# liuzhenboo/Stereo-Visual-Odometry

Hardware: AMD Instinct MI355X
Metric: stereo frames/sec on KITTI-00 1241x376; LK-kernel achieved HBM GB/s vs peak (higher is better)
Workload: dtype u8; 1 GPU; S0 synthetic KITTI-like stereo sequence 1241x376 (config #2 stand-in), FAST+LK track_mode LK_stereof2f_pnp, batched frame pairs (256 per step, 4 distinct chunks cycled), frames resident in HBM for `value`; `m1` (--full) = host-resident frames, H2D included; pairs_ok_last_step=256, parallelism=1 GPU

## Files before the change

include/svo_abi.h:

```cpp
#ifndef SVO_ABI_H
#define SVO_ABI_H

#include <stdint.h>

#ifdef __cplusplus
extern "C" {
#endif

#define SVO_ABI_VERSION 9

#define SVO_OK                 0
#define SVO_ERR_ARG           -1
#define SVO_ERR_HIP           -2
#define SVO_ERR_NOMEM         -3
#define SVO_ERR_STATE         -4
#define SVO_FAIL_FEW_KEYPOINTS 1
#define SVO_FAIL_FEW_TRACKS    2
#define SVO_FAIL_INLIER_RATIO  3
#define SVO_FAIL_ROTATION_GATE 4
#define SVO_FAIL_TRANSL_GATE   5
#define SVO_FAIL_CAPACITY      6

#define SVO_MEM_HOST   0
#define SVO_MEM_DEVICE 1

typedef struct svo_ctx svo_ctx;

typedef struct { float x, y; } svo_pt2f;
typedef struct { float x, y, z; } svo_pt3f;
typedef struct {
    float x, y, size, angle, response;
    int32_t octave, class_id;
} svo_keypoint;

typedef struct {
    int32_t width, height;
    int32_t max_keypoints;
    int32_t max_batch;
    int32_t num_slots;
    int32_t fast_threshold;
    int32_t num_features_tracking;
    int32_t iterations;
    float   reproj_err;
    float   confidence;
    double  feature_match_error;
    double  inlier_rate;
    double  min_move2, max_move2;
    double  P1[12], P2[12];
    int32_t track_mode;
    int32_t orb_nfeatures;
    float   orb_scale_factor;
    int32_t orb_nlevels;
    int32_t orb_ini_th, orb_min_th;
    int32_t lk_accum;
    int32_t fast_keep_strongest;
} svo_config;

#define SVO_MODE_LK  0
#define SVO_MODE_ORB 1
#define SVO_LK_ACCUM_EXACT 0
#define SVO_LK_ACCUM_SSE2  1
#define SVO_LK_ACCUM_SIMD128 2
#define SVO_LK_ACCUM_SSE2_LEGACY 3

typedef struct {
    double rvec[3], tvec[3], R[9];
    int32_t n_inliers, ransac_iters, best_iter, lm_iters, ok, _pad;
} svo_pnp_result;

typedef struct {
    int32_t ok;
    int32_t fail_stage;
    int32_t n_prev_kps, n_cur_kps, n_tracked, n_inliers;
    int32_t ransac_iters, lm_iters;
    double  rvec[3], tvec[3], R[9];
    double  T_rel_inv[16];
    double  pose[16];
} svo_step_result;

int         svo_abi_version(void);
int         svo_config_bytes(void);
void        svo_default_config(svo_config *cfg, int width, int height);
int         svo_device_count(int *n);
int         svo_create(const svo_config *cfg, int device, svo_ctx **out);
void        svo_destroy(svo_ctx *ctx);
const char *svo_last_error(const svo_ctx *ctx);
int         svo_set_stream(svo_ctx *ctx, void *hip_stream);
int         svo_sync(svo_ctx *ctx);
int         svo_wait_stream(svo_ctx *ctx, void *hip_stream);
int         svo_signal_stream(svo_ctx *ctx, void *hip_stream);
int         svo_signal_stream_inputs(svo_ctx *ctx, void *hip_stream);
int         svo_num_levels(const svo_ctx *ctx);


int svo_fast_detect(svo_ctx *ctx, const uint8_t *img, int pitch, int mem, int threshold,
                    int nonmax, svo_keypoint *out, int cap, int *n_out);

int svo_build_pyramid(svo_ctx *ctx, int slot, const uint8_t *img, int pitch, int mem);
int svo_read_pyramid_level(svo_ctx *ctx, int slot, int level, uint8_t *out, int out_pitch, int mem,
                           int *w, int *h);

int svo_lk_track(svo_ctx *ctx, int slot_prev, int slot_next, const svo_pt2f *prev_pts, int n,
                 svo_pt2f *next_pts, uint8_t *status, int mem);

int svo_circular_match(svo_ctx *ctx, int slot_prevL, int slot_prevR, int slot_curL, int slot_curR,
                       const svo_pt2f *t1_left, int n, svo_pt2f *out_t1_left,
                       svo_pt2f *out_t1_right, svo_pt2f *out_t2_right, svo_pt2f *out_t2_left,
                       int *m_out, int mem);

int svo_triangulate(svo_ctx *ctx, const double P1[12], const double P2[12], const svo_pt2f *x1,
                    const svo_pt2f *x2, int n, svo_pt3f *out, int mem);

int svo_pnp_ransac(svo_ctx *ctx, const svo_pt3f *obj, const svo_pt2f *img, int n, const double K[9],
                   int iterations, float reproj_err, double confidence, svo_pnp_result *res,
                   uint8_t *inlier_mask, int mem);

int svo_orb_extract(svo_ctx *ctx, const uint8_t *img, int pitch, int mem, svo_keypoint *kps, uint8_t *desc,
                    int cap, int *n_out, int *per_level);
int svo_orb_read_level(svo_ctx *ctx, int level, uint8_t *out, int *w, int *h);
int svo_orb_read_candidates(svo_ctx *ctx, int level, float *out4, int cap, int *n_out);

int svo_match_hamming(svo_ctx *ctx, const uint8_t *query, int nq, const uint8_t *train, int nt, int32_t *train_idx,
                      float *distance, int mem);


int svo_add_frame(svo_ctx *ctx, const uint8_t *left, const uint8_t *right, int pitch, int mem,
                  svo_step_result *res);
int svo_reset(svo_ctx *ctx);
int svo_get_pose(svo_ctx *ctx, double pose[16]);
int svo_set_pose(svo_ctx *ctx, const double pose[16]);

int svo_track_batch(svo_ctx *ctx, const uint8_t *left_frames, const uint8_t *right_frames,
                    int pitch, int64_t frame_stride, int n_frames, const double *pose0,
                    svo_step_result *results, int results_mem);

int svo_set_overlap(svo_ctx *ctx, int on);
int svo_wait_results(svo_ctx *ctx);

int svo_host_alloc(svo_ctx *ctx, size_t bytes, void **out);
int svo_host_free(svo_ctx *ctx, void *p);
int svo_upload_frames(svo_ctx *ctx, int buf, const uint8_t *left_frames, const uint8_t *right_frames,
                      int pitch, int64_t frame_stride, int n_frames);
int svo_upload_frames_at(svo_ctx *ctx, int buf, int first_slot, const uint8_t *left_frames, const uint8_t *right_frames,
                         int pitch, int64_t frame_stride, int n_frames);
int svo_wait_upload(svo_ctx *ctx, int buf);
int svo_track_uploaded(svo_ctx *ctx, int buf, int n_frames, const double *pose0,
                       svo_step_result *results, int results_mem);
#define SVO_CONTINUE_CHAIN       1
#define SVO_CONTINUE_CARRY_FRAME 2
int svo_track_uploaded_async(svo_ctx *ctx, int buf, int n_frames, const double *pose0, int continue_chain);
int svo_collect_results(svo_ctx *ctx, svo_step_result *results, int n_pairs);
int svo_results_ready(svo_ctx *ctx, int *n_pairs);

int svo_get_frame_keypoints(svo_ctx *ctx, int side, svo_keypoint *kps, uint8_t *descriptors, int cap, int *n_out);
int svo_get_last_tracks(svo_ctx *ctx, svo_pt2f *t1_left, svo_pt2f *t1_right, svo_pt2f *t2_right,
                        svo_pt2f *t2_left, uint8_t *inlier, int cap, int *n_out);
int svo_get_batch_tracks(svo_ctx *ctx, int pair, svo_pt2f *t1_left, svo_pt2f *t1_right, svo_pt2f *t2_right,
                         svo_pt2f *t2_left, uint8_t *inlier, int cap, int *n_out);

int svo_streams_create(svo_ctx *ctx, int n_streams);
int svo_streams_count(const svo_ctx *ctx, int *n_streams);
int svo_streams_step(svo_ctx *ctx, const int32_t *stream_ids, int m, const uint8_t *left_frames,
                     const uint8_t *right_frames, int pitch, int64_t frame_stride, int mem,
                     svo_step_result *results, int results_mem);
int svo_streams_reset(svo_ctx *ctx, int stream_id);
int svo_streams_get_pose(svo_ctx *ctx, int stream_id, double pose[16]);
int svo_streams_set_pose(svo_ctx *ctx, int stream_id, const double pose[16]);
int svo_streams_get_tracks(svo_ctx *ctx, int item, svo_pt2f *t1_left, svo_pt2f *t1_right, svo_pt2f *t2_right,
                           svo_pt2f *t2_left, uint8_t *inlier, int cap, int *n_out);

#define SVO_INTERP_NEAREST 0
#define SVO_INTERP_LINEAR  1
int svo_scale_projection(const double P[12], double inv_x, double inv_y, int interp, double P_out[12]);
int svo_resize(svo_ctx *ctx, const uint8_t *src, int sw, int sh, int spitch, int64_t sstride,
               uint8_t *dst, int dw, int dh, int dpitch, int64_t dstride, int n_frames,
               int interp, double fx, double fy, int mem);
int svo_ingest_create(svo_ctx *ctx, int src_width, int src_height, int interp, double fx, double fy);
int svo_ingest_info(const svo_ctx *ctx, int *src_width, int *src_height, int *interp, double *inv_x, double *inv_y);
int svo_ingest_add_frame(svo_ctx *ctx, const uint8_t *left, const uint8_t *right, int pitch, int mem, svo_step_result *res);
int svo_ingest_track_batch(svo_ctx *ctx, const uint8_t *lefts, const uint8_t *rights, int pitch, int64_t frame_stride,
                           int n_frames, const double *pose0, svo_step_result *results, int results_mem);
int svo_ingest_streams_step(svo_ctx *ctx, const int32_t *stream_ids, int m, const uint8_t *lefts, const uint8_t *rights,
                            int pitch, int64_t frame_stride, int mem, svo_step_result *results, int results_mem);
// ... 57 lines not shown
```

stereo-visual-odometry_amd/binding.py:

```python
import ctypes as C
import os
import subprocess

import numpy as np

_HERE = os.path.dirname(os.path.abspath(__file__))
_LIB = None

MEM_HOST, MEM_DEVICE = 0, 1

KP_DTYPE = np.dtype([("x", "<f4"), ("y", "<f4"), ("size", "<f4"), ("angle", "<f4"),
                     ("response", "<f4"), ("octave", "<i4"), ("class_id", "<i4")])


class SvoError(RuntimeError):
    pass


class Config(C.Structure):
    _fields_ = [("width", C.c_int32), ("height", C.c_int32), ("max_keypoints", C.c_int32),
                ("max_batch", C.c_int32), ("num_slots", C.c_int32), ("fast_threshold", C.c_int32),
                ("num_features_tracking", C.c_int32), ("iterations", C.c_int32),
                ("reproj_err", C.c_float), ("confidence", C.c_float),
                ("feature_match_error", C.c_double), ("inlier_rate", C.c_double),
# ... 230 lines not shown
        return rc

    def sync(self):
        self._check(self.lib.svo_sync(self.h))

    def set_stream(self, stream_handle):
        self._check(self.lib.svo_set_stream(self.h, C.c_void_p(stream_handle)))
        self._stream_handle = int(stream_handle or 0)

    def wait_stream(self, stream_handle):
        self._check(self.lib.svo_wait_stream(self.h, C.c_void_p(stream_handle)))

    def signal_stream(self, stream_handle):
        self._check(self.lib.svo_signal_stream(self.h, C.c_void_p(stream_handle)))

    def signal_stream_inputs(self, stream_handle):
        self._check(self.lib.svo_signal_stream_inputs(self.h, C.c_void_p(stream_handle)))

    def _order_in(self, t):
        import torch
        other = torch.cuda.current_stream(t.device).cuda_stream
        if other and other == getattr(self, "_stream_handle", 0):
            return False
        self.wait_stream(other)
        return True

    def _order_out(self, t):
        import torch
        other = torch.cuda.current_stream(t.device).cuda_stream
        if other and other == getattr(self, "_stream_handle", 0):
            return
        self.signal_stream(other)

    @property
    def num_levels(self):
        return self.lib.svo_num_levels(self.h)

    def set_overlap(self, on=True):
        self._check(self.lib.svo_set_overlap(self.h, int(on)))

    def wait_results(self):
        self._check(self.lib.svo_wait_results(self.h))

    def enable_timing(self, on=True):
        self._check(self.lib.svo_enable_timing(self.h, int(on)))

    def get_timing(self):
        names = (C.c_char_p * 64)()
        ms = (C.c_float * 64)()
        n = self.lib.svo_get_timing(self.h, names, ms, 64)
        return [(names[i].decode(), float(ms[i])) for i in range(n)]

    def _img(self, img, shape=None):
        shape = shape or (self.height, self.width)
        assert tuple(img.shape) == tuple(shape), (tuple(img.shape), shape)
        if isinstance(img, np.ndarray):
            assert img.dtype == np.uint8 and img.strides[1] == 1
            return C.c_void_p(img.ctypes.data), int(img.strides[0]), MEM_HOST
        assert img.element_size() == 1 and img.stride(1) == 1
        return C.c_void_p(img.data_ptr()), int(img.stride(0)), (MEM_DEVICE if img.is_cuda else MEM_HOST)

    def fast_detect(self, img, threshold=20, nonmax=True, cap=None):
        cap = cap or self.cfg.max_keypoints
        p, pitch, mem = self._img(img)
        out = np.zeros(cap, dtype=KP_DTYPE)
        n = C.c_int(0)
        self._check(self.lib.svo_fast_detect(self.h, p, pitch, mem, int(threshold), int(bool(nonmax)),
                                             C.c_void_p(out.ctypes.data), cap, C.byref(n)))
        return out[:n.value].copy()

    def build_pyramid(self, slot, img):
        p, pitch, mem = self._img(img)
        self._check(self.lib.svo_build_pyramid(self.h, int(slot), p, pitch, mem))

    def read_pyramid_level(self, slot, level):
        w, h = C.c_int(0), C.c_int(0)
        self._check(self.lib.svo_read_pyramid_level(self.h, slot, level, None, 0, MEM_HOST,
                                                    C.byref(w), C.byref(h)))
        out = np.zeros((h.value, w.value), np.uint8)
        self._check(self.lib.svo_read_pyramid_level(self.h, slot, level, C.c_void_p(out.ctypes.data),
                                                    w.value, MEM_HOST, C.byref(w), C.byref(h)))
        return out

    def lk_track(self, slot_prev, slot_next, pts):
        if isinstance(pts, np.ndarray):
            pts = np.ascontiguousarray(pts, np.float32).reshape(-1, 2)
            n = pts.shape[0]
            out = np.zeros((n, 2), np.float32)
            st = np.zeros(n, np.uint8)
        else:
            import torch
            n = pts.shape[0]
            out = torch.zeros((n, 2), dtype=torch.float32, device=pts.device)
            st = torch.zeros(n, dtype=torch.uint8, device=pts.device)
            self._order_in(st)
        pi, mem = _ptr(pts)
        po, _ = _ptr(out)
        ps, _ = _ptr(st)
        self._check(self.lib.svo_lk_track(self.h, slot_prev, slot_next, pi, n, po, ps, mem))
        if mem == MEM_DEVICE:
            self._order_out(st)
        return out, st

    def circular_match(self, slots, t1_left):
        if isinstance(t1_left, np.ndarray):
            t1_left = np.ascontiguousarray(t1_left, np.float32).reshape(-1, 2)
            n = t1_left.shape[0]
            outs = [np.zeros((max(n, 1), 2), np.float32) for _ in range(4)]
        else:
            import torch
            n = t1_left.shape[0]
            outs = [torch.zeros((max(n, 1), 2), dtype=torch.float32, device=t1_left.device) for _ in range(4)]
            self._order_in(outs[0])
        pi, mem = _ptr(t1_left)
        m = C.c_int(0)
        self._check(self.lib.svo_circular_match(self.h, *[int(s) for s in slots], pi, n,
                                                *[_ptr(o)[0] for o in outs], C.byref(m), mem))
        return [o[:m.value] for o in outs]

    def triangulate(self, P1, P2, x1, x2):
        P1 = np.ascontiguousarray(P1, np.float64).reshape(12)
        P2 = np.ascontiguousarray(P2, np.float64).reshape(12)
        if isinstance(x1, np.ndarray):
            x1 = np.ascontiguousarray(x1, np.float32).reshape(-1, 2)
            x2 = np.ascontiguousarray(x2, np.float32).reshape(-1, 2)
            out = np.zeros((x1.shape[0], 3), np.float32)
        else:
            import torch
            out = torch.zeros((x1.shape[0], 3), dtype=torch.float32, device=x1.device)
            self._order_in(out)
        p1, mem = _ptr(x1)
        p2, _ = _ptr(x2)
        self._check(self.lib.svo_triangulate(self.h, C.c_void_p(P1.ctypes.data), C.c_void_p(P2.ctypes.data),
                                             p1, p2, x1.shape[0], _ptr(out)[0], mem))
        if mem == MEM_DEVICE:
            self._order_out(out)
        return out

    def pnp_ransac(self, obj, img, K, iterations=500, reproj_err=0.5, confidence=0.99):
        K = np.ascontiguousarray(K, np.float64).reshape(9)
        if isinstance(obj, np.ndarray):
            obj = np.ascontiguousarray(obj, np.float32).reshape(-1, 3)
            img = np.ascontiguousarray(img, np.float32).reshape(-1, 2)
            mask = np.zeros(max(obj.shape[0], 1), np.uint8)
        else:
            import torch
            mask = torch.zeros(max(obj.shape[0], 1), dtype=torch.uint8, device=obj.device)
            self._order_in(mask)
        n = obj.shape[0]
        res = PnPResult()
        po, mem = _ptr(obj)
        conf = float(np.float32(confidence))
        self._check(self.lib.svo_pnp_ransac(self.h, po, _ptr(img)[0], n, C.c_void_p(K.ctypes.data),
                                            int(iterations), C.c_float(reproj_err), C.c_double(conf),
                                            C.byref(res), _ptr(mask)[0], mem))
        if mem == MEM_DEVICE:
            self._order_out(mask)
            mask = mask.cpu().numpy()
        return dict(ok=res.ok, rvec=np.array(res.rvec), tvec=np.array(res.tvec),
                    R=np.array(res.R).reshape(3, 3), n_inliers=res.n_inliers,
                    ransac_iters=res.ransac_iters, best_iter=res.best_iter, lm_iters=res.lm_iters,
                    mask=np.asarray(mask[:n]).copy())

    def set_pose_refine(self, mode, rounds=4, iters=10, sigma_px=1.0, min_inliers=6):
        names = {"off": REFINE_OFF, "none": REFINE_OFF, "reproj": REFINE_REPROJ}
        m = names[mode] if isinstance(mode, str) and mode in names else mode
# ... 488 lines not shown
```

stereo-visual-odometry_amd/csrc/fast.hip:

```cpp
#include "svo_device.h"
#include "svo_kernels.h"

namespace svo {

constexpr int kTileW = 64, kTileH = 16, kHalo = 4;
constexpr int kRawW = kTileW + 2 * kHalo;
constexpr int kRawH = kTileH + 2 * kHalo;
constexpr int kScW = kTileW + 2;
constexpr int kScH = kTileH + 2;

__device__ __forceinline__ void load_circle(const uint8_t *c, int d[16], int v)
{
    constexpr int P = kRawW;
    d[0] = v - c[3 * P];       d[1] = v - c[3 * P + 1];   d[2] = v - c[2 * P + 2];   d[3] = v - c[P + 3];
    d[4] = v - c[3];           d[5] = v - c[-P + 3];      d[6] = v - c[-2 * P + 2];  d[7] = v - c[-3 * P + 1];
    d[8] = v - c[-3 * P];      d[9] = v - c[-3 * P - 1];  d[10] = v - c[-2 * P - 2]; d[11] = v - c[-P - 3];
    d[12] = v - c[-3];         d[13] = v - c[P - 3];      d[14] = v - c[2 * P - 2];  d[15] = v - c[3 * P - 1];
}

__device__ __forceinline__ bool has_arc9(unsigned m16)
{
    unsigned m = m16 | (m16 << 16);
    unsigned a = m & (m >> 1);
    unsigned b = a & (a >> 2);
// ... 106 lines not shown
#pragma unroll
                for (int hb = 0; hb < 2; hb++) {
                    auto half = [&](uint32_t w) { return __builtin_bit_cast(s16x2, (hb ? w >> 8 : w) & 0x00FF00FFu); };
                    const s16x2 v = half(C), u = half(U), d = half(D), l = half(Lv), rr = half(Rv);
                    const s16x2 mnA = __builtin_elementwise_min(u, d), mxA = __builtin_elementwise_max(u, d);
                    const s16x2 mnB = __builtin_elementwise_min(l, rr), mxB = __builtin_elementwise_max(l, rr);
                    const s16x2 dark = __builtin_elementwise_min(v - mnA, v - mnB);
                    const s16x2 bright = __builtin_elementwise_min(mxA - v, mxB - v);
                    sgn[hb] = __builtin_bit_cast(uint32_t, __builtin_elementwise_max(dark, bright) - T1);
                }
                const uint32_t dead = ((sgn[0] >> 15) & 1u) | ((sgn[1] >> 14) & 2u) | ((sgn[0] >> 29) & 4u) | ((sgn[1] >> 28) & 8u);
                const int gy = y0 - 1 + sy, gxb = x0 - 1 + sxb;
                const int lo = max(max(0, -sxb), 3 - gxb), hi = min(min(4, kScW - sxb), a.w - 3 - gxb);
                const uint32_t inside = (hi > lo && gy >= 3 && gy < a.h - 3) ? ((1u << hi) - 1u) & ~((1u << lo) - 1u) : 0u;
                m4 = ~dead & inside;
            }
            const int lane = threadIdx.x;
            const unsigned long long lt = (1ull << lane) - 1ull;
            const unsigned long long b0 = __ballot(m4 & 1u), b1 = __ballot(m4 & 2u), b2 = __ballot(m4 & 4u), b3 = __ballot(m4 & 8u);
            const int c0 = __popcll(b0), c1 = __popcll(b1), c2 = __popcll(b2), c3 = __popcll(b3);
            if (c0 + c1 + c2 + c3) {
                int base = 0;
                if (lane == 0) base = atomicAdd(&n_cand, c0 + c1 + c2 + c3);
                base = __builtin_amdgcn_readfirstlane(base);
                const int pos = sy * kScW + sxb;
                if (m4 & 1u) cand[base + __popcll(b0 & lt)] = (uint16_t)pos;
                if (m4 & 2u) cand[base + c0 + __popcll(b1 & lt)] = (uint16_t)(pos + 1);
                if (m4 & 4u) cand[base + c0 + c1 + __popcll(b2 & lt)] = (uint16_t)(pos + 2);
                if (m4 & 8u) cand[base + c0 + c1 + c2 + __popcll(b3 & lt)] = (uint16_t)(pos + 3);
            }
        }
    }
    __syncthreads();
    const int nc = n_cand;
    for (int i0 = 0; i0 < nc; i0 += 256) {
        const int i = i0 + tid;
        const int pos = i < nc ? cand[i] : 0;
        const int sy = pos / kScW, sx = pos - sy * kScW;
        const bool corner = i < nc && fast_arc(&raw[(sy + kHalo - 1) * kRawW + sx + kHalo - 1], a.thr);
        if (a.nms) list_push(corner, pos, corners, &n_corner);
        else if (corner) sc[pos] = 1;
    }
    __syncthreads();
    if (a.nms) {
        const int nk = n_corner;
        for (int i = tid; i < nk; i += 256) {
            const int pos = corners[i];
            const int sy = pos / kScW, sx = pos - sy * kScW;
            sc[pos] = (uint8_t)fast_corner_score(&raw[(sy + kHalo - 1) * kRawW + sx + kHalo - 1], a.thr);
        }
        __syncthreads();
    }

#pragma unroll
    for (int j = 0; j < kTileH / 4; j++) {
        int ly = threadIdx.y + 4 * j, lx = threadIdx.x;
        int gx = x0 + lx, gy = y0 + ly;
        const uint8_t *p = &sc[(ly + 1) * kScW + lx + 1];
        int s = p[0];
        if (a.nms && s) {
            bool keep = s > p[-1] && s > p[1] && s > p[-kScW - 1] && s > p[-kScW] && s > p[-kScW + 1] &&
                        s > p[kScW - 1] && s > p[kScW] && s > p[kScW + 1];
            if (!keep) s = 0;
        }
        bool inimg = gx < a.w && gy < a.h;
        if (!inimg) s = 0;
        unsigned long long m = __ballot(s != 0);
        if (inimg) score[(int64_t)gy * a.spitch + gx] = (uint8_t)s;
        if (threadIdx.x == 0 && m && gy < a.h) atomicAdd(&rowcount[gy], __popcll(m));
    }
}

__global__ __launch_bounds__(256) void fast_emit_kernel(FastArgs a)
{
    const int b = blockIdx.y;
    const int y = blockIdx.x * 4 + (threadIdx.x >> 6);
    const int lane = threadIdx.x & 63;
    if (y >= a.h) return;
    const uint8_t *score = a.score + (int64_t)b * a.score_stride + (int64_t)y * a.spitch;
    const int *rowcount = a.rowcount + (int64_t)b * a.rowcount_stride;
    int mine = rowcount[y];
    bool last = (y == a.h - 1);
    if (mine == 0 && !last) return;
    int part = 0;
    for (int r = lane; r < y; r += 64) part += rowcount[r];
    int off = wave_sum_i32(part);
    if (last && lane == 0) a.n_out[b] = off + mine;
    if (mine == 0) return;
    float2 *xy = a.kp_xy + (int64_t)b * a.kp_stride;
    float *resp = a.kp_resp + (int64_t)b * a.kp_stride;
    for (int x = lane; x < ((a.w + 63) & ~63); x += 64) {
        int s = x < a.w ? score[x] : 0;
        unsigned long long m = __ballot(s != 0);
        if (s) {
            int idx = off + __popcll(m & ((1ull << lane) - 1ull));
            if (idx < a.cap) {
                xy[idx] = make_float2((float)x, (float)y);
                resp[idx] = a.nms ? (float)s : 0.f;
            }
        }
        off += __popcll(m);
    }
}

__global__ __launch_bounds__(1024) void fast_keep_strongest_kernel(FastArgs a, int keep)
{
    __shared__ int hist[256];
    __shared__ int wave_eq[16], wave_kp[16];
    __shared__ int s_t, s_need_eq, s_eq_base, s_out_base;
    const int b = blockIdx.x, tid = threadIdx.x, lane = tid & 63, wv = tid >> 6;
    const int n = a.n_out[b];
    if (n <= keep || n > a.cap) return;
    float2 *xy = a.kp_xy + (int64_t)b * a.kp_stride;
    float *resp = a.kp_resp + (int64_t)b * a.kp_stride;
    if (tid < 256) hist[tid] = 0;
    __syncthreads();
    for (int i = tid; i < n; i += 1024) atomicAdd(&hist[min(255, max(0, (int)resp[i]))], 1);
    __syncthreads();
    if (tid == 0) {
        int above = 0, t = 255;
        for (; t > 0; t--) {
            if (above + hist[t] >= keep) break;
            above += hist[t];
        }
        s_t = t; s_need_eq = keep - above; s_eq_base = 0; s_out_base = 0;
    }
    __syncthreads();
    const int t = s_t, need_eq = s_need_eq;
    for (int start = 0; start < n; start += 1024) {
        const int i = start + tid;
        const bool in = i < n;
        const float2 p = in ? xy[i] : make_float2(0.f, 0.f);
        const float r = in ? resp[i] : 0.f;
        const int ri = (int)r;
        const bool eq = in && ri == t;
        const unsigned long long me = __ballot(eq);
        if (lane == 0) wave_eq[wv] = __popcll(me);
        __syncthreads();
        int eq_pre = s_eq_base, eq_tot = 0;
        for (int q = 0; q < 16; q++) { const int c = wave_eq[q]; if (q < wv) eq_pre += c; eq_tot += c; }
        const int eq_rank = eq_pre + __popcll(me & ((1ull << lane) - 1ull));
        const bool kp = in && (ri > t || (eq && eq_rank < need_eq));
        const unsigned long long mk = __ballot(kp);
        if (lane == 0) wave_kp[wv] = __popcll(mk);
        __syncthreads();
        int kp_pre = s_out_base, kp_tot = 0;
        for (int q = 0; q < 16; q++) { const int c = wave_kp[q]; if (q < wv) kp_pre += c; kp_tot += c; }
        if (kp) {
            const int dst = kp_pre + __popcll(mk & ((1ull << lane) - 1ull));
            xy[dst] = p; resp[dst] = r;
        }
        __syncthreads();
        if (tid == 0) { s_eq_base += eq_tot; s_out_base += kp_tot; }
        __syncthreads();
    }
    if (tid == 0) a.n_out[b] = keep;
}

void launch_fast_keep_strongest(const FastArgs &a, int batch, int keep, hipStream_t st)
{
    if (keep <= 0 || batch <= 0 || !a.nms) return;
    hipLaunchKernelGGL(fast_keep_strongest_kernel, dim3(batch), dim3(1024), 0, st, a, keep);
}

constexpr int kBucketLdsCells = 3072;

__device__ __forceinline__ void bucket_count(int *cnt, int cell, bool flag)
{
    const int lane = threadIdx.x & 63;
    const int prev = __shfl_up(cell, 1);
    const bool head = lane == 0 || prev != cell;
    const unsigned long long H = __ballot(head), F = __ballot(flag);
    if (head && cell >= 0) {
        const unsigned long long below = (1ull << lane) - 1ull;
        const unsigned long long after = lane == 63 ? 0ull : H & ~(below | (1ull << lane));
        const unsigned long long upto = after ? (1ull << (__ffsll((long long)after) - 1)) - 1ull : ~0ull;
        const int c = __popcll(F & upto & ~below);
        if (c) atomicAdd(&cnt[4 * cell], c);
    }
}

template <bool kLds>
__global__ __launch_bounds__(1024) void fast_bucket_kernel(BucketArgs a)
{
// ... 128 lines not shown
```

stereo-visual-odometry_amd/csrc/pyramid.hip:

```cpp
#include "svo_device.h"
#include "svo_kernels.h"

namespace svo {

__device__ __forceinline__ const uint8_t *src_image(const PyrArgs &a, int b)
{
    if (a.img2) return ((b & 1) ? a.img2 : a.img) + (int64_t)(b >> 1) * a.img_stride;
    return a.img + (int64_t)b * a.img_stride;
}

__global__ __launch_bounds__(256) void pyr_copy0_kernel(PyrArgs a)
{
    const int b = blockIdx.z, y = blockIdx.y * blockDim.y + threadIdx.y;
    const int w = a.g.w[0];
    if (y >= a.g.h[0]) return;
    const uint8_t *src = src_image(a, b) + (int64_t)y * a.pitch;
    uint8_t *dst = a.slots + (int64_t)b * a.slot_stride + a.g.origin[0] + (int64_t)y * a.g.pitch[0];
    const int x = (blockIdx.x * blockDim.x + threadIdx.x) * 16;
    if (x >= w) return;
    if (x + 16 <= w && ((uintptr_t)(src + x) & 15) == 0) {
        *(uint4 *)(dst + x) = *(const uint4 *)(src + x);
    } else {
        for (int q = 0; q < 16 && x + q < w; q++) dst[x + q] = src[x + q];
    }
}

constexpr int kBorderRows = 16;
constexpr int kFrameRowsPerWg = 4, kSidePasses = 4;
__host__ __device__ inline int border_top_groups() { return 2 * kPad / kFrameRowsPerWg; }
__host__ __device__ inline int border_side_groups(int h) { return (h + kBorderRows * kSidePasses - 1) / (kBorderRows * kSidePasses); }
__global__ __launch_bounds__(256) void pyr_border_kernel(PyrArgs a, int l)
{
    const int b = blockIdx.y;
    const int w = a.g.w[l], h = a.g.h[l], pitch = a.g.pitch[l];
    uint8_t *lvl = a.slots + (int64_t)b * a.slot_stride + a.g.origin[l];
    if ((int)blockIdx.x < border_top_groups()) {
        for (int q = 0; q < kFrameRowsPerWg; q++) {
            const int gidx = blockIdx.x * kFrameRowsPerWg + q;
            const int py = gidx < kPad ? gidx - kPad : h + (gidx - kPad);
            const uint8_t *src = lvl + (int64_t)refl101(py, h) * pitch;
            uint8_t *dst = lvl + (int64_t)py * pitch;
            for (int px = ((int)threadIdx.x << 2) - kPad; px < w + kPad; px += 1024) {
                uint32_t v = 0;
                if (px >= 0 && px + 4 <= w) v = *(const uint32_t *)(src + px);
                else {
#pragma unroll
                    for (int k = 0; k < 4; k++) v |= (uint32_t)src[refl101(min(px + k, w + kPad - 1), w)] << (8 * k);
                }
                if (px + 4 <= w + kPad) *(uint32_t *)(dst + px) = v;
                else for (int k = 0; px + k < w + kPad; k++) dst[px + k] = (uint8_t)(v >> (8 * k));
            }
        }
        return;
    }
    const int sgroup = blockIdx.x - border_top_groups();
    if (w >= 2 * kPad) {
        static_assert(kBorderRows == 16 && kPad == 32, "256 threads = 16 rows x 16 dwords");
        typedef uint32_t u32_unaligned __attribute__((aligned(1)));
        const int k = threadIdx.x & 15, r = threadIdx.x >> 4;
        const int px = k < 8 ? -kPad + 4 * k : w + 4 * (k - 8);
        const int c0 = k < 8 ? kPad - 3 - 4 * k : w - 5 - 4 * (k - 8);
        for (int q = 0; q < kSidePasses; q++) {
            const int py = (sgroup * kSidePasses + q) * kBorderRows + r;
            if (py >= h) return;
            uint8_t *row = lvl + (int64_t)py * pitch;
            const uint32_t v = *(const u32_unaligned *)(row + c0);
            *(u32_unaligned *)(row + px) = __builtin_amdgcn_perm(0u, v, 0x00010203u);
        }
    } else {
        const int t = threadIdx.x & 63;
        const int px = t < kPad ? t - kPad : w + (t - kPad);
        const int sx = refl101(px, w);
        for (int q = 0; q < kSidePasses; q++)
            for (int r = threadIdx.x >> 6; r < kBorderRows; r += 4) {
                const int py = (sgroup * kSidePasses + q) * kBorderRows + r;
                if (py >= h) return;
                uint8_t *row = lvl + (int64_t)py * pitch;
                row[px] = row[sx];
            }
    }
}

__global__ __launch_bounds__(256) void pyr_down_kernel(PyrArgs a, int l)
{
    const int b = blockIdx.z, y = blockIdx.y * blockDim.y + threadIdx.y;
    const int w = a.g.w[l];
    if (y >= a.g.h[l]) return;
    const int sp = a.g.pitch[l - 1];
    uint8_t *slot = a.slots + (int64_t)b * a.slot_stride;
    const uint8_t *src = slot + a.g.origin[l - 1];
    uint8_t *dst = slot + a.g.origin[l] + (int64_t)y * a.g.pitch[l];
    const int x0 = (blockIdx.x * blockDim.x + threadIdx.x) * 4;
    if (x0 >= w) return;
    int acc[4] = {0, 0, 0, 0};
#pragma unroll
    for (int r = 0; r < 5; r++) {
        const uint32_t *row = (const uint32_t *)(src + (int64_t)(2 * y + r - 2) * sp + 2 * x0 - 4);
        const uint32_t d0 = row[0], d1 = row[1], d2 = row[2], d3 = row[3];
        int s[16];
#pragma unroll
        for (int j = 0; j < 4; j++) {
            s[j] = (d0 >> (8 * j)) & 255; s[4 + j] = (d1 >> (8 * j)) & 255;
            s[8 + j] = (d2 >> (8 * j)) & 255; s[12 + j] = (d3 >> (8 * j)) & 255;
        }
        const int wv = (r == 2) ? 6 : ((r == 1 || r == 3) ? 4 : 1);
#pragma unroll
        for (int q = 0; q < 4; q++) {
            const int c = 4 + 2 * q;
            const int hs = s[c] * 6 + (s[c - 1] + s[c + 1]) * 4 + s[c - 2] + s[c + 2];
            acc[q] += hs * wv;
        }
    }
    uint32_t out = 0;
#pragma unroll
    for (int q = 0; q < 4; q++) out |= (uint32_t)((acc[q] + 128) >> 8) << (8 * q);
    if (x0 + 4 <= w) *(uint32_t *)(dst + x0) = out;
    else for (int q = 0; x0 + q < w; q++) dst[x0 + q] = (uint8_t)(out >> (8 * q));
}

__global__ __launch_bounds__(256) void pyr_read_level_kernel(PyrGeom g, const uint8_t *slot, int l,
                                                              uint8_t *out, int out_pitch)
{
    int x = blockIdx.x * 256 + threadIdx.x, y = blockIdx.y;
    if (x >= g.w[l]) return;
    out[(int64_t)y * out_pitch + x] = slot[g.origin[l] + (int64_t)y * g.pitch[l] + x];
}

void launch_pyramid(const PyrArgs &a, int batch, hipStream_t st)
{
    dim3 blk(256, 1, 1);
    auto shape = [](int lanes_per_row, int rows, dim3 &grid, dim3 &block, int batch) {
        const int bx = lanes_per_row < 256 ? lanes_per_row : 256, by = 256 / bx;
        block = dim3(bx, by, 1);
        grid = dim3((lanes_per_row + bx - 1) / bx, (rows + by - 1) / by, batch);
    };
    {
        dim3 g, bk;
        shape((a.g.w[0] + 15) / 16, a.g.h[0], g, bk, batch);
        hipLaunchKernelGGL(pyr_copy0_kernel, g, bk, 0, st, a);
    }
    for (int l = 0; l < a.g.nlevels; l++) {
        if (l > 0) {
            dim3 g, bk;
            shape((a.g.w[l] + 3) / 4, a.g.h[l], g, bk, batch);
            hipLaunchKernelGGL(pyr_down_kernel, g, bk, 0, st, a, l);
        }
        dim3 gb(border_top_groups() + border_side_groups(a.g.h[l]), batch, 1);
        hipLaunchKernelGGL(pyr_border_kernel, gb, blk, 0, st, a, l);
    }
}

// ... 9 lines not shown
```

stereo-visual-odometry_amd/csrc/svo_abi.hip:

```cpp
#include <algorithm>
#include <cmath>
#include <cstdio>
#include <cstring>
#include <ctime>
#include <new>
#include <vector>
#include "abi_io.h"

using namespace svo;

namespace svo {
int dev_alloc_raw(svo_ctx *ctx, void **out, size_t bytes)
{
    *out = nullptr;
    if (bytes == 0) bytes = 1;
    if (ctx->arena.planning) {
        ctx->arena.plan.emplace_back(out, ctx->arena.planned);
        ctx->arena.planned += align_up(bytes, kDevAlign);
        return SVO_OK;
    }
    SVO_HIP(hipMalloc(out, bytes));
    ctx->arena.extra.push_back(*out);
    return SVO_OK;
}
// ... 387 lines not shown
    SVO_ARG(img != nullptr, "null image");
    SVO_ARG(pitch >= ctx->cfg.width, "pitch < width");
    if (mem == SVO_MEM_DEVICE) { *dptr = img; *dpitch = pitch; return SVO_OK; }
    SVO_ARG(mem == SVO_MEM_HOST, "mem must be SVO_MEM_HOST or SVO_MEM_DEVICE");
    return svo::stage_host_image(ctx, img, pitch, stage_idx, dptr, dpitch);
}

extern "C" int svo_fast_detect(svo_ctx *ctx, const uint8_t *img, int pitch, int mem, int threshold,
                               int nonmax, svo_keypoint *out, int cap, int *n_out)
{
    if (!ctx) return SVO_ERR_ARG;
    SVO_ARG(out && n_out && cap >= 0, "null output");
    SVO_HIP(hipSetDevice(ctx->device));
    const uint8_t *d; int dp;
    int rc = resolve_image(ctx, img, pitch, mem, 0, &d, &dp);
    if (rc) return rc;
    FastArgs a{};
    a.img = d; a.pitch = dp; a.img_stride = 0;
    a.w = ctx->cfg.width; a.h = ctx->cfg.height;
    a.thr = threshold < 0 ? 0 : (threshold > 255 ? 255 : threshold);
    a.nms = nonmax != 0;
    a.score = ctx->score; a.spitch = ctx->spitch; a.score_stride = ctx->score_stride;
    a.rowcount = ctx->rowcount; a.rowcount_stride = ctx->rowcount_stride;
    a.kp_xy = ctx->kp_xy; a.kp_resp = ctx->kp_resp; a.kp_stride = ctx->cfg.max_keypoints;
    a.n_out = ctx->kp_n; a.cap = ctx->cfg.max_keypoints;
    launch_fast(a, 1, ctx->stream);
    SVO_HIP(hipGetLastError());
    int n;
    SVO_TRY(count_read(ctx, ctx->kp_n, &n));
    *n_out = n;
    if (n > ctx->cfg.max_keypoints) { ctx->err = "FAST: keypoints exceed max_keypoints"; return SVO_ERR_ARG; }
    if (n > cap) { ctx->err = "FAST: keypoints exceed caller capacity"; return SVO_ERR_ARG; }
    if (n == 0) return SVO_OK;
    float2 *h_xy;
    SVO_TRY(pinned_block(ctx, (sizeof(float2) + sizeof(float)) * (size_t)ctx->cfg.max_keypoints, &h_xy));
    float *h_r = (float *)(h_xy + ctx->cfg.max_keypoints);
    SVO_TRY(from_device(ctx, h_xy, (const float2 *)ctx->kp_xy, (size_t)n, SVO_MEM_HOST));
    SVO_TRY(from_device(ctx, h_r, (const float *)ctx->kp_resp, (size_t)n, SVO_MEM_HOST));
    SVO_TRY(io_done(ctx, SVO_MEM_HOST));
    format_keypoints(h_xy, h_r, n, out);
    return SVO_OK;
}

extern "C" int svo_build_pyramid(svo_ctx *ctx, int slot, const uint8_t *img, int pitch, int mem)
{
    if (!ctx) return SVO_ERR_ARG;
    SVO_ARG(slot >= 0 && slot < ctx->cfg.num_slots, "slot out of range");
    SVO_HIP(hipSetDevice(ctx->device));
    const uint8_t *d; int dp;
    int rc = resolve_image(ctx, img, pitch, mem, 0, &d, &dp);
    if (rc) return rc;
    PyrArgs a{};
    a.g = ctx->geom; a.img = d; a.pitch = dp; a.img_stride = 0;
    a.slots = ctx->slots + (size_t)slot * ctx->geom.slot_bytes; a.slot_stride = 0;
    launch_pyramid(a, 1, ctx->stream);
    SVO_HIP(hipGetLastError());
    if (mem == SVO_MEM_HOST) SVO_HIP(hipStreamSynchronize(ctx->stream));
    ctx->slot_built[slot] = 1;
    return SVO_OK;
}

extern "C" int svo_read_pyramid_level(svo_ctx *ctx, int slot, int level, uint8_t *out, int out_pitch,
                                      int mem, int *w, int *h)
{
    if (!ctx) return SVO_ERR_ARG;
    SVO_ARG(slot >= 0 && slot < ctx->cfg.num_slots, "slot out of range");
    SVO_ARG(level >= 0 && level < ctx->geom.nlevels, "level out of range");
    if (!ctx->slot_built[slot]) { ctx->err = "pyramid slot not built"; return SVO_ERR_STATE; }
    const int lw = ctx->geom.w[level], lh = ctx->geom.h[level];
    if (w) *w = lw;
    if (h) *h = lh;
    if (!out) return SVO_OK;
    SVO_ARG(out_pitch >= lw, "out_pitch < level width");
    SVO_HIP(hipSetDevice(ctx->device));
    const uint8_t *s = ctx->slots + (size_t)slot * ctx->geom.slot_bytes;
    if (mem == SVO_MEM_DEVICE) {
        launch_pyr_read_level(ctx->geom, s, level, out, out_pitch, ctx->stream);
        SVO_HIP(hipGetLastError());
        return SVO_OK;
    }
    SVO_HIP(hipMemcpy2DAsync(out, out_pitch, s + ctx->geom.origin[level], ctx->geom.pitch[level], lw, lh,
                             hipMemcpyDeviceToHost, ctx->stream));
    SVO_HIP(hipStreamSynchronize(ctx->stream));
    return SVO_OK;
}

static void fill_lk_common(svo_ctx *ctx, LkArgs &a, int n)
{
    a.g = ctx->geom;
    a.slot_stride = 0;
    a.pts_stride = 0;
    a.n_pts = nullptr; a.n_fixed = n; a.cap = n;
    a.match_err = ctx->cfg.feature_match_error;
    a.accum = ctx->cfg.lk_accum;
}

extern "C" int svo_lk_track(svo_ctx *ctx, int slot_prev, int slot_next, const svo_pt2f *prev_pts, int n,
                            svo_pt2f *next_pts, uint8_t *status, int mem)
{
    if (!ctx) return SVO_ERR_ARG;
    SVO_ARG(slot_prev >= 0 && slot_prev < ctx->cfg.num_slots && slot_next >= 0 &&
            slot_next < ctx->cfg.num_slots, "slot out of range");
    SVO_ARG(n >= 0 && n <= ctx->cfg.max_keypoints, "n exceeds max_keypoints");
    SVO_ARG(mem == SVO_MEM_HOST || mem == SVO_MEM_DEVICE, "bad mem");
    if (!ctx->slot_built[slot_prev] || !ctx->slot_built[slot_next]) { ctx->err = "pyramid slot not built"; return SVO_ERR_STATE; }
    if (n == 0) return SVO_OK;
    SVO_ARG(prev_pts && next_pts && status, "null pointer");
    SVO_HIP(hipSetDevice(ctx->device));
    const float2 *d_in;
    SVO_TRY(to_device(ctx, (const float2 *)prev_pts, ctx->pts_in, (size_t)n, mem, &d_in));
    LkArgs a{};
    fill_lk_common(ctx, a, n);
    a.ncalls = 1;
    a.prev[0] = ctx->slots + (size_t)slot_prev * ctx->geom.slot_bytes;
    a.next[0] = ctx->slots + (size_t)slot_next * ctx->geom.slot_bytes;
    a.pts_in = d_in;
    a.pts_out[0] = mem == SVO_MEM_DEVICE ? (float2 *)next_pts : ctx->pts_out[0];
    a.status[0] = mem == SVO_MEM_DEVICE ? status : ctx->status[0];
    launch_lk(a, 1, n, ctx->stream);
    SVO_HIP(hipGetLastError());
    SVO_TRY(from_device(ctx, (float2 *)next_pts, (const float2 *)a.pts_out[0], (size_t)n, mem));
    SVO_TRY(from_device(ctx, status, (const uint8_t *)a.status[0], (size_t)n, mem));
    return io_done(ctx, mem);
}

extern "C" int svo_circular_match(svo_ctx *ctx, int slot_prevL, int slot_prevR, int slot_curL, int slot_curR,
                                  const svo_pt2f *t1_left, int n, svo_pt2f *out_t1_left,
                                  svo_pt2f *out_t1_right, svo_pt2f *out_t2_right, svo_pt2f *out_t2_left,
                                  int *m_out, int mem)
{
    if (!ctx) return SVO_ERR_ARG;
    const int sl[4] = {slot_prevL, slot_prevR, slot_curL, slot_curR};
    for (int i = 0; i < 4; i++) {
        SVO_ARG(sl[i] >= 0 && sl[i] < ctx->cfg.num_slots, "slot out of range");
        if (!ctx->slot_built[sl[i]]) { ctx->err = "pyramid slot not built"; return SVO_ERR_STATE; }
    }
    SVO_ARG(n >= 0 && n <= ctx->cfg.max_keypoints, "n exceeds max_keypoints");
    SVO_ARG(mem == SVO_MEM_HOST || mem == SVO_MEM_DEVICE, "bad mem");
    SVO_ARG(m_out != nullptr, "null m_out");
    if (svo_wait_results(ctx) != SVO_OK) return SVO_ERR_HIP;
    *m_out = 0;
    if (n == 0) return SVO_OK;
    SVO_ARG(t1_left && out_t1_left && out_t1_right && out_t2_right && out_t2_left, "null pointer");
    SVO_HIP(hipSetDevice(ctx->device));
    const float2 *d_in;
    SVO_TRY(to_device(ctx, (const float2 *)t1_left, ctx->pts_in, (size_t)n, mem, &d_in));
    auto S = [&](int s) { return ctx->slots + (size_t)s * ctx->geom.slot_bytes; };
    LkArgs a{};
    fill_lk_common(ctx, a, n);
    a.ncalls = 4;
    a.prev[0] = S(slot_prevL); a.next[0] = S(slot_prevR);
    a.prev[1] = S(slot_prevR); a.next[1] = S(slot_curR);
    a.prev[2] = S(slot_curR);  a.next[2] = S(slot_curL);
    a.prev[3] = S(slot_curL);  a.next[3] = S(slot_prevL);
    a.pts_in = d_in;
    for (int i = 0; i < 4; i++) { a.pts_out[i] = ctx->pts_out[i]; a.status[i] = ctx->status[i]; }
    a.keep = ctx->keep;
    launch_lk(a, 1, n, ctx->stream);
    CompactArgs c{};
    c.keep = ctx->keep; c.n_pts = nullptr; c.n_fixed = n; c.pts_stride = 0; c.cap = n;
    c.in[0] = d_in; c.in[1] = ctx->pts_out[0]; c.in[2] = ctx->pts_out[1]; c.in[3] = ctx->pts_out[2];
    svo_pt2f *outs[4] = {out_t1_left, out_t1_right, out_t2_right, out_t2_left};
    for (int i = 0; i < 4; i++) c.out[i] = mem == SVO_MEM_DEVICE ? (float2 *)outs[i] : ctx->cmp[i];
    c.m_out = ctx->m_out;
    launch_compact(c, 1, ctx->stream);
    SVO_HIP(hipGetLastError());
// ... 973 lines not shown
```

Measured before the change: 19570 stereo pairs/s.

## Vectorize FAST emit scans and pyramid border reflection with wide loads

The FAST emit kernel now reads score rows as 4-byte words, preloading five trips per lane ahead of the prefix-sum. It compacts keypoints with a wave inclusive scan over per-lane counts instead of a per-byte ballot. Pyramid border padding now copies 16-byte pieces: top and bottom rows are filled with 128-bit vector copies, and the reflected side strips use 16-byte byte-reversed loads and stores instead of 4-byte perms. A padded pyramid-level readback API is also added for debugging or validation. The wide accesses are unaligned and add more masking logic, so edge-case correctness at row tails matters.

After: 19660 stereo pairs/s (median of 6 runs). About the same (+0.5%).

```diff
diff --git a/include/svo_abi.h b/include/svo_abi.h
--- a/include/svo_abi.h
+++ b/include/svo_abi.h
@@ -99,6 +99,8 @@
 int svo_build_pyramid(svo_ctx *ctx, int slot, const uint8_t *img, int pitch, int mem);
 int svo_read_pyramid_level(svo_ctx *ctx, int slot, int level, uint8_t *out, int out_pitch, int mem,
                            int *w, int *h);
+int svo_read_pyramid_level_padded(svo_ctx *ctx, int slot, int level, uint8_t *out, int out_pitch, int mem,
+                                  int *w, int *h, int *pad);
 
 int svo_lk_track(svo_ctx *ctx, int slot_prev, int slot_next, const svo_pt2f *prev_pts, int n,
                  svo_pt2f *next_pts, uint8_t *status, int mem);
diff --git a/stereo-visual-odometry_amd/binding.py b/stereo-visual-odometry_amd/binding.py
--- a/stereo-visual-odometry_amd/binding.py
+++ b/stereo-visual-odometry_amd/binding.py
@@ -336,6 +336,15 @@
                                                     w.value, MEM_HOST, C.byref(w), C.byref(h)))
         return out
 
+    def read_pyramid_level_padded(self, slot, level):
+        w, h, pad = C.c_int(0), C.c_int(0), C.c_int(0)
+        self._check(self.lib.svo_read_pyramid_level_padded(self.h, slot, level, None, 0, MEM_HOST,
+                                                           C.byref(w), C.byref(h), C.byref(pad)))
+        out = np.zeros((h.value, w.value), np.uint8)
+        self._check(self.lib.svo_read_pyramid_level_padded(self.h, slot, level, C.c_void_p(out.ctypes.data),
+                                                           w.value, MEM_HOST, C.byref(w), C.byref(h), C.byref(pad)))
+        return out, pad.value
+
     def lk_track(self, slot_prev, slot_next, pts):
         if isinstance(pts, np.ndarray):
             pts = np.ascontiguousarray(pts, np.float32).reshape(-1, 2)
diff --git a/stereo-visual-odometry_amd/csrc/fast.hip b/stereo-visual-odometry_amd/csrc/fast.hip
--- a/stereo-visual-odometry_amd/csrc/fast.hip
+++ b/stereo-visual-odometry_amd/csrc/fast.hip
@@ -212,6 +212,20 @@
     int mine = rowcount[y];
     bool last = (y == a.h - 1);
     if (mine == 0 && !last) return;
+    constexpr int kEmitTrips = 5;
+    const bool dwords = (((uintptr_t)score | (uintptr_t)a.spitch) & 3) == 0;
+    auto load4 = [&](int x) -> uint32_t {
+        uint32_t v = 0;
+        if (x < a.w) {
+            if (dwords && x + 4 <= a.spitch) v = *(const uint32_t *)(score + x);
+            else for (int k = 0; k < 4 && x + k < a.w; k++) v |= (uint32_t)score[x + k] << (8 * k);
+            if (x + 4 > a.w) v &= 0xFFFFFFFFu >> (8 * (x + 4 - a.w));
+        }
+        return v;
+    };
+    uint32_t v[kEmitTrips];
+#pragma unroll
+    for (int t = 0; t < kEmitTrips; t++) v[t] = mine ? load4(256 * t + 4 * lane) : 0u;
     int part = 0;
     for (int r = lane; r < y; r += 64) part += rowcount[r];
     int off = wave_sum_i32(part);
@@ -219,17 +233,34 @@
     if (mine == 0) return;
     float2 *xy = a.kp_xy + (int64_t)b * a.kp_stride;
     float *resp = a.kp_resp + (int64_t)b * a.kp_stride;
-    for (int x = lane; x < ((a.w + 63) & ~63); x += 64) {
-        int s = x < a.w ? score[x] : 0;
-        unsigned long long m = __ballot(s != 0);
-        if (s) {
-            int idx = off + __popcll(m & ((1ull << lane) - 1ull));
-            if (idx < a.cap) {
-                xy[idx] = make_float2((float)x, (float)y);
-                resp[idx] = a.nms ? (float)s : 0.f;
+    for (int xb = 0; xb < a.w; xb += 256 * kEmitTrips) {
+        if (xb) {
+#pragma unroll
+            for (int t = 0; t < kEmitTrips; t++) v[t] = load4(xb + 256 * t + 4 * lane);
+        }
+#pragma unroll
+        for (int t = 0; t < kEmitTrips; t++) {
+            if (xb + 256 * t >= a.w) break;
+            const int x = xb + 256 * t + 4 * lane;
+            const uint32_t q = v[t];
+            const int cnt = (int)((q & 0xFFu) != 0) + (int)((q & 0xFF00u) != 0) + (int)((q & 0xFF0000u) != 0) + (int)((q >> 24) != 0);
+            const int incl = wave_incl_scan(cnt);
+            int idx = off + incl - cnt;
+            if (cnt) {
+#pragma unroll
+                for (int k = 0; k < 4; k++) {
+                    const int sk = (q >> (8 * k)) & 255;
+                    if (sk) {
+                        if (idx < a.cap) {
+                            xy[idx] = make_float2((float)(x + k), (float)y);
+                            resp[idx] = a.nms ? (float)sk : 0.f;
+                        }
+                        idx++;
+                    }
+                }
             }
-        }
-        off += __popcll(m);
+            off += __builtin_amdgcn_readlane(incl, 63);
+        }
     }
 }
 
diff --git a/stereo-visual-odometry_amd/csrc/pyramid.hip b/stereo-visual-odometry_amd/csrc/pyramid.hip
--- a/stereo-visual-odometry_amd/csrc/pyramid.hip
+++ b/stereo-visual-odometry_amd/csrc/pyramid.hip
@@ -29,12 +29,55 @@
 constexpr int kFrameRowsPerWg = 4, kSidePasses = 4;
 __host__ __device__ inline int border_top_groups() { return 2 * kPad / kFrameRowsPerWg; }
 __host__ __device__ inline int border_side_groups(int h) { return (h + kBorderRows * kSidePasses - 1) / (kBorderRows * kSidePasses); }
+
+typedef uint32_t u32x4 __attribute__((ext_vector_type(4)));
+typedef u32x4 u32x4_unaligned __attribute__((aligned(1)));
+__device__ __forceinline__ u32x4 bytes_reversed(u32x4 v)
+{
+    return u32x4{__builtin_bswap32(v.w), __builtin_bswap32(v.z), __builtin_bswap32(v.y), __builtin_bswap32(v.x)};
+}
+__device__ __forceinline__ void side_piece(int k, int w, int &sx, int &dx)
+{
+    sx = k == 0 ? kPad - 15 : k == 1 ? 1 : k == 2 ? w - 17 : w - 33;
+    dx = k == 0 ? -kPad : k == 1 ? -16 : k == 2 ? w : w + 16;
+}
+
 __global__ __launch_bounds__(256) void pyr_border_kernel(PyrArgs a, int l)
 {
+    static_assert(kPad == 32, "two 16-byte pieces per side");
     const int b = blockIdx.y;
     const int w = a.g.w[l], h = a.g.h[l], pitch = a.g.pitch[l];
     uint8_t *lvl = a.slots + (int64_t)b * a.slot_stride + a.g.origin[l];
+    const bool wide = w >= 2 * kPad;
     if ((int)blockIdx.x < border_top_groups()) {
+        if (wide) {
+            static_assert(kFrameRowsPerWg == 4, "256 threads = 4 waves = 4 frame rows");
+            const int lane = threadIdx.x & 63;
+            const int gidx = blockIdx.x * kFrameRowsPerWg + (threadIdx.x >> 6);
+            const int py = gidx < kPad ? gidx - kPad : h + (gidx - kPad);
+            const uint8_t *src = lvl + (int64_t)refl101(py, h) * pitch;
+            uint8_t *dst = lvl + (int64_t)py * pitch;
+            const int nfull = w >> 4, ntail = (w & 15) ? 1 : 0, npieces = nfull + ntail + 4;
+            for (int i0 = lane; i0 < npieces; i0 += 128) {
+                u32x4 v[2];
+                int dx[2];
+                bool on[2], rev[2];
+#pragma unroll
+                for (int t = 0; t < 2; t++) {
+                    const int i = i0 + 64 * t;
+                    int sx = 0;
+                    on[t] = i < npieces;
+                    rev[t] = i >= nfull + ntail;
+                    if (rev[t]) side_piece(i - nfull - ntail, w, sx, dx[t]);
+                    else sx = dx[t] = i < nfull ? 16 * i : w - 16;
+                    if (on[t]) v[t] = *(const u32x4_unaligned *)(src + sx);
+                }
+#pragma unroll
+                for (int t = 0; t < 2; t++)
+                    if (on[t]) *(u32x4_unaligned *)(dst + dx[t]) = rev[t] ? bytes_reversed(v[t]) : v[t];
+            }
+            return;
+        }
         for (int q = 0; q < kFrameRowsPerWg; q++) {
             const int gidx = blockIdx.x * kFrameRowsPerWg + q;
             const int py = gidx < kPad ? gidx - kPad : h + (gidx - kPad);
@@ -54,19 +97,15 @@
         return;
     }
     const int sgroup = blockIdx.x - border_top_groups();
-    if (w >= 2 * kPad) {
-        static_assert(kBorderRows == 16 && kPad == 32, "256 threads = 16 rows x 16 dwords");
-        typedef uint32_t u32_unaligned __attribute__((aligned(1)));
-        const int k = threadIdx.x & 15, r = threadIdx.x >> 4;
-        const int px = k < 8 ? -kPad + 4 * k : w + 4 * (k - 8);
-        const int c0 = k < 8 ? kPad - 3 - 4 * k : w - 5 - 4 * (k - 8);
-        for (int q = 0; q < kSidePasses; q++) {
-            const int py = (sgroup * kSidePasses + q) * kBorderRows + r;
-            if (py >= h) return;
-            uint8_t *row = lvl + (int64_t)py * pitch;
-            const uint32_t v = *(const u32_unaligned *)(row + c0);
-            *(u32_unaligned *)(row + px) = __builtin_amdgcn_perm(0u, v, 0x00010203u);
-        }
+    if (wide) {
+        static_assert(kBorderRows * kSidePasses * 4 == 256, "256 threads = 64 rows x 4 pieces");
+        const int py = sgroup * (kBorderRows * kSidePasses) + ((int)threadIdx.x >> 2);
+        if (py >= h) return;
+        uint8_t *row = lvl + (int64_t)py * pitch;
+        int sx, dx;
+        side_piece(threadIdx.x & 3, w, sx, dx);
+        const u32x4 v = *(const u32x4_unaligned *)(row + sx);
+        *(u32x4_unaligned *)(row + dx) = bytes_reversed(v);
     } else {
         const int t = threadIdx.x & 63;
         const int px = t < kPad ? t - kPad : w + (t - kPad);
diff --git a/stereo-visual-odometry_amd/csrc/svo_abi.hip b/stereo-visual-odometry_amd/csrc/svo_abi.hip
--- a/stereo-visual-odometry_amd/csrc/svo_abi.hip
+++ b/stereo-visual-odometry_amd/csrc/svo_abi.hip
@@ -493,6 +493,28 @@
     SVO_HIP(hipMemcpy2DAsync(out, out_pitch, s + ctx->geom.origin[level], ctx->geom.pitch[level], lw, lh,
                              hipMemcpyDeviceToHost, ctx->stream));
     SVO_HIP(hipStreamSynchronize(ctx->stream));
+    return SVO_OK;
+}
+
+extern "C" int svo_read_pyramid_level_padded(svo_ctx *ctx, int slot, int level, uint8_t *out, int out_pitch,
+                                             int mem, int *w, int *h, int *pad)
+{
+    if (!ctx) return SVO_ERR_ARG;
+    SVO_ARG(slot >= 0 && slot < ctx->cfg.num_slots, "slot out of range");
+    SVO_ARG(level >= 0 && level < ctx->geom.nlevels, "level out of range");
+    if (!ctx->slot_built[slot]) { ctx->err = "pyramid slot not built"; return SVO_ERR_STATE; }
+    const int pw = ctx->geom.w[level] + 2 * kPad, ph = ctx->geom.h[level] + 2 * kPad;
+    if (w) *w = pw;
+    if (h) *h = ph;
+    if (pad) *pad = kPad;
+    if (!out) return SVO_OK;
+    SVO_ARG(out_pitch >= pw, "out_pitch < padded level width");
+    SVO_HIP(hipSetDevice(ctx->device));
+    const uint8_t *s = ctx->slots + (size_t)slot * ctx->geom.slot_bytes + ctx->geom.origin[level] -
+                       ((int64_t)kPad * ctx->geom.pitch[level] + kPad);
+    SVO_HIP(hipMemcpy2DAsync(out, out_pitch, s, ctx->geom.pitch[level], pw, ph,
+                             mem == SVO_MEM_DEVICE ? hipMemcpyDeviceToDevice : hipMemcpyDeviceToHost, ctx->stream));
+    if (mem != SVO_MEM_DEVICE) SVO_HIP(hipStreamSynchronize(ctx->stream));
     return SVO_OK;
 }
 
```
